# 0xPolygonZero/proof-protocol-decoder

Hardware: AMD Instinct MI355X
Metric: txn-proofs/sec (whole node), 256-txn synthetic block (higher is better)
Workload: dtype u64 (Goldilocks field)

## Files before the change

### include/bpg.h

```cpp
#ifndef BPG_H
#define BPG_H
#include <stddef.h>
#include <stdint.h>

#ifdef __cplusplus
extern "C" {
#endif

typedef enum {
  BP_OK = 0,
  BP_ERR_ABORTED = -1,
  BP_ERR_INVALID_INPUT = -2,
  BP_ERR_RANGE = -3,
  BP_ERR_DEVICE = -4,
  BP_ERR_VERIFY = -5,
  BP_ERR_UNSUPPORTED = -6
} bp_status;

const char* bp_last_error(void);
const char* bp_version(void);
int bp_device_count(void);
int bp_use_blocking_sync(int device);
int bp_host_wait_mode(int device);

// ... 127 lines not shown
typedef struct bp_plonk_layout {
  uint32_t pi_len, n_paths, path_depth, path_pi0;
  uint32_t leaf_len;
} bp_plonk_layout;
int bp_plonk_constants(uint64_t seed, uint32_t log_n, const bp_plonk_layout* layout, uint64_t* d_consts_out, void* stream);
int bp_plonk_trace(const uint64_t* d_consts, uint64_t seed, const uint64_t* pi, const bp_plonk_layout* layout, const uint64_t* paths,
                   uint32_t log_n, uint64_t* d_trace_out, void* stream);

int bp_fri_fold(const uint64_t* d_values, uint32_t log_nl, uint32_t rate_bits, uint32_t arity_bits, uint64_t shift,
                const uint64_t beta[2], uint64_t* d_out, void* stream);

int bp_openings(const uint64_t* d_coeffs, uint64_t stride, uint32_t log_n, uint32_t n_cols, const uint64_t z0[2],
                const uint64_t z1[2], uint64_t* d_pw_scratch, uint64_t* d_out, void* stream);

int bp_pow_grind(const uint64_t state[12], uint32_t pos, uint32_t bits, uint64_t* nonce_out, void* stream);

typedef struct bp_stark_cfg {
  uint32_t log_n, n_cols, n_const, deg_pow, rate_bits, cap_height, num_queries, pow_bits, arity_bits,
      final_poly_bits;
} bp_stark_cfg;
int bp_stark_prove_synthetic(const bp_stark_cfg* cfg, uint64_t seed, uint64_t const_seed, int device,
                             uint8_t** out, size_t* out_len);
int bp_stark_prove_air(uint32_t air_id, const bp_stark_cfg* cfg, uint64_t seed, uint64_t const_seed, int device,
                       uint8_t** out, size_t* out_len);
int bp_stark_prove_trace(uint32_t air_id, const bp_stark_cfg* cfg, const uint64_t* d_trace, uint64_t stride,
                         const uint64_t* d_consts, const uint64_t* pub, int device, uint8_t** out, size_t* out_len);
int bp_stark_verify_air(uint32_t air_id, const bp_stark_cfg* cfg, const uint64_t* const_cap, const uint8_t* proof,
                        size_t len);
void bp_stark_public_inputs(uint64_t seed, uint64_t out[4]);
void bp_stark_public_input_list(uint64_t seed, uint64_t out[4]);
// ... 220 lines not shown
```

### proof_protocol_decoder_amd/_abi.py

```python
import ctypes as C
from ctypes import POINTER as P

vp, cp, i, sz, dbl = C.c_void_p, C.c_char_p, C.c_int, C.c_size_t, C.c_double
u8, u32, u64, i32, i64 = C.c_uint8, C.c_uint32, C.c_uint64, C.c_int32, C.c_int64
u8p, u32p, u64p, i32p, szp = P(u8), P(u32), P(u64), P(i32), P(sz)
u8pp = P(u8p)

BP_OK, BP_ERR_ABORTED, BP_ERR_INVALID_INPUT, BP_ERR_RANGE, BP_ERR_DEVICE, BP_ERR_VERIFY, BP_ERR_UNSUPPORTED = 0, -1, -2, -3, -4, -5, -6
STATUS_NAMES = {v: k for k, v in list(globals().items()) if k == "BP_OK" or k.startswith("BP_ERR_")}
BP_SET_SKIP_LINK_CHECK = 1
BP_NUM_TABLES, BP_IR_WORDS, BP_PV_WORDS = 7, 25, 13

KNOBS = ("quad_threshold", "assume_loaded", "merkle_fused", "merkle_wide", "poseidon_mx", "poseidon_mx_sets",
         "poseidon_grouped", "ntt_mx", "ntt_split", "k5_spread", "host_wait", "host_poseidon", "rec_batch",
         "witness_threads", "side_lanes")


def _u32s(*names):
    return [(n, u32) for n in names]


class AirFamily(C.Structure):
    _fields_ = _u32s("first_index", "count", "kind", "degree")

# ... 170 lines not shown
    "bp_arithmetic_div_trace": (i, [vp, u32, vp, vp]),
    "bp_arithmetic_div_layout": (i, [u32p, sz]),
    "bp_arithmetic_mod_trace": (i, [vp, u32, vp, vp]),
    "bp_arithmetic_mod_layout": (i, [u32p, sz]),
    "bp_arithmetic_shift_trace": (i, [vp, u32, vp, vp]),
    "bp_arithmetic_shift_layout": (i, [u32p, sz]),
    "bp_arithmetic_sdiv_trace": (i, [vp, u32, vp, vp]),
    "bp_arithmetic_sdiv_layout": (i, [u32p, sz]),
    "bp_arithmetic_exp_trace": (i, [vp, u32, vp, u32, vp, vp]),
    "bp_arithmetic_exp_layout": (i, [u32p, sz]),
    "bp_plonk_constants": (i, [u64, u32, P(PlonkLayout), vp, vp]),
    "bp_plonk_trace": (i, [vp, u64, u64p, P(PlonkLayout), u64p, u32, vp, vp]),
    "bp_fri_fold": (i, [vp, u32, u32, u32, u64, u64p, vp, vp]),
    "bp_openings": (i, [vp, u64, u32, u32, u64p, u64p, vp, vp, vp]),
    "bp_pow_grind": (i, [u64p, u32, u32, u64p, vp]),
    "bp_stark_prove_synthetic": (i, [_cfg, u64, u64, i] + _buf),
    "bp_stark_prove_air": (i, [u32, _cfg, u64, u64, i] + _buf),
    "bp_stark_prove_trace": (i, [u32, _cfg, vp, u64, vp, u64p, i] + _buf),
    "bp_stark_verify_air": (i, [u32, _cfg, u64p, cp, sz]),
    "bp_stark_public_inputs": (None, [u64, u64p]),
    "bp_stark_public_input_list": (None, [u64, u64p]),
    "bp_stark_verify_air_pub": (i, [u32, _cfg, u64p, u64p, cp, sz]),
    "bp_stark_prove_table_set": (i, [P(SetTable), u32, P(SetLink), u32, u32, i] + _buf),
    "bp_stark_verify_table_set": (i, [P(SetTable), u32, P(u64p), P(SetLink), u32, cp, sz]),
    "bp_check_table_set": (i, [P(SetTable), u32, P(SetLink), u32, i, P(SetReport)]),
    "bp_release_cached_memory": (None, []),
    "bp_free_buffer": (None, [u8p]),
    "bp_config_default": (None, [_conf]),
    "bp_state_build": (i, [_conf, P(vp)]),
    "bp_state_free": (None, [vp]),
# ... 54 lines not shown
```

### proof_protocol_decoder_amd/csrc/poseidon.cuh

```cuda
#pragma once
#include "gl.hpp"
#include "mx_arith.cuh"

namespace poseidon {

static __constant__ uint64_t RC[360] = {
#include "poseidon_rc.inc"
};

__device__ __forceinline__ uint64_t sbox(uint64_t x) {
  uint64_t x2 = gl::sqr(x);
  uint64_t x4 = gl::sqr(x2);
  uint64_t x3 = gl::mul(x2, x);
  return gl::mul(x3, x4);
}

template <int N>
__device__ __forceinline__ void sbox_n(uint64_t (&x)[N]) {
  uint64_t x2[N], x4[N], x3[N];
  gl::mul_n<N>(x, x, x2);
  gl::mul_n<N>(x2, x2, x4);
  gl::mul_n<N>(x2, x, x3);
  gl::mul_n<N>(x3, x4, x);
}
// ... 37 lines not shown
        L[rr] += (uint64_t)lo[(i + r) % 12] * C[i];
        H[rr] += (uint64_t)hi[(i + r) % 12] * C[i];
      }
      if (r == 0) {
        L[rr] += (uint64_t)lo[0] * 8;
        H[rr] += (uint64_t)hi[0] * 8;
      }
    }
    uint64_t out[4];
    reduce_rows<4>(L, H, out);
#pragma unroll
    for (int rr = 0; rr < 4; rr++) s[4 * g + rr] = out[rr];
  }
}

__device__ __forceinline__ void permute(uint64_t (&s)[12]) {
#pragma unroll
  for (int i = 0; i < 12; i++) s[i] = gl::add(s[i], RC[i]);
  int rnd = 0;
#pragma unroll 1
  for (int k = 0; k < 4; k++, rnd++) {
    sbox_all(s);
    mds<true>(s, RC + (rnd + 1) * 12);
  }
#pragma unroll 1
  for (int k = 0; k < 22; k++, rnd++) {
    s[0] = sbox(s[0]);
    mds<true>(s, RC + (rnd + 1) * 12);
  }
#pragma unroll 1
  for (int k = 0; k < 3; k++, rnd++) {
    sbox_all(s);
    mds<true>(s, RC + (rnd + 1) * 12);
  }
  sbox_all(s);
  mds<false>(s, nullptr);
}
// ... 93 lines not shown
```

### proof_protocol_decoder_amd/csrc/poseidon_mx.cuh

```cuda
#pragma once
#include "poseidon.cuh"
#include "poseidon_group.hpp"

namespace poseidon {
namespace mx {

using mxa::v4i;

constexpr int CIN_PER_ROUND = 4 * 24;
constexpr int CIN_WORDS = 30 * CIN_PER_ROUND;

__device__ __forceinline__ uint32_t mds_entry(uint32_t i, uint32_t k) {
  constexpr uint32_t C[12] = {17, 15, 41, 16, 2, 28, 13, 13, 39, 18, 34, 20};
  const uint32_t d = (k + 12 - i) % 12;
  uint32_t v = 0;
#pragma unroll
  for (int j = 0; j < 12; j++) v = d == (uint32_t)j ? C[j] : v;
  return v + ((i | k) == 0 ? 8u : 0u);
}

struct CinTable {
  uint32_t v[CIN_WORDS];
};
constexpr CinTable make_cin_table() {
// ... 342 lines not shown
    blo[3] = 0;
    bhi[3] = 0;
    uint64_t L[3], H[3];
#pragma unroll
    for (int g = 0; g < 3; g++) {
      const v4i A = am[g * 64];
      const v4i dl = __builtin_amdgcn_mfma_i32_16x16x64_i8(A, blo, cr[2 * g], 0, 0, 0);
      const v4i dh = __builtin_amdgcn_mfma_i32_16x16x64_i8(A, bhi, cr[2 * g + 1], 0, 0, 0);
      L[g] = planes(dl);
      H[g] = planes(dh);
    }
    reduce_rows<3>(L, H, e[m]);
  }
}

__device__ __forceinline__ void permute_grouped(uint64_t (&e)[4][3], const Ctx& c, const uint32_t* tab,
                                                const uint32_t* __restrict__ gtab) {
#pragma unroll
  for (int a = 0; a < 3; a++) {
    const uint64_t k = RC[c.kb + 4 * a];
#pragma unroll
    for (int m = 0; m < 4; m++) e[m][a] = gl::add(e[m][a], k);
  }
  int rnd = 0;
#pragma unroll 1
  for (int k = 0; k < 4; k++, rnd++) {
    sbox_full<4>(e);
    mds4_lds(e, c, rnd, tab);
  }
  grp::State s;
  grp::init_state(s);
  grp::Lanes o = grp::lanes_of(threadIdx.x & 63);
#pragma unroll 1
  for (int g = 0; g < grp::N_GROUPS; g++) grp::partial_group(s, o, e, tab, gtab, g);
  rnd = 26;
#pragma unroll 1
  for (int k = 0; k < 4; k++, rnd++) {
    sbox_full<4>(e);
    mds4_lds(e, c, rnd, tab);
  }
}

template <int NS>
__device__ __forceinline__ void permute(uint64_t (&e)[NS][3], const Ctx& c) {
#pragma unroll
  for (int a = 0; a < 3; a++) {
    const uint64_t k = RC[c.kb + 4 * a];
#pragma unroll
    for (int m = 0; m < NS; m++) e[m][a] = gl::add(e[m][a], k);
  }
  int rnd = 0;
#pragma unroll 1
  for (int k = 0; k < 4; k++, rnd++) {
    sbox_full<NS>(e);
    mds<NS>(e, c, rnd);
  }
#pragma unroll 1
  for (int k = 0; k < 22; k++, rnd++) {
    sbox_word0<NS>(e, c);
    mds<NS>(e, c, rnd);
  }
#pragma unroll 1
  for (int k = 0; k < 4; k++, rnd++) {
    sbox_full<NS>(e);
    mds<NS>(e, c, rnd);
  }
}

}
}
```

### proof_protocol_decoder_amd/csrc/prover.cpp

```cpp
#include <cstdio>
#include <cstdlib>
#include "prover.hpp"
#include "tune.hpp"
#include <algorithm>
#include <chrono>
#if defined(__x86_64__)
#include <immintrin.h>
#endif
#include <memory>
#include <mutex>
#include <unordered_map>
#include <thread>

namespace bpg {

static const uint64_t RC_HOST[360] = {
#include "poseidon_rc.inc"
};
static inline uint64_t sbox_host(uint64_t x) {
  uint64_t x2 = gl::mulc(x, x), x4 = gl::mulc(x2, x2), x3 = gl::mulc(x2, x);
  return gl::mulc(x3, x4);
}
static const uint32_t MDS_C[12] = {17, 15, 41, 16, 2, 28, 13, 13, 39, 18, 34, 20};
static inline void mds_finish_host(const uint64_t al[12], const uint64_t ah[12], uint64_t s[12]) {
// ... 67 lines not shown
      else for (int i = 0; i < 12; i++) s[i] = sbox_host(s[i]);
      mds(s);
    }
  }
}
#if defined(__x86_64__)
__attribute__((target("avx2"))) static void poseidon_host_avx2(uint64_t s[12]) { poseidon_host_body<true>(s); }
#endif
static void poseidon_host_scalar(uint64_t s[12]) { poseidon_host_body<false>(s); }
void poseidon_host(uint64_t s[12]) {
#if defined(__x86_64__)
  static const bool avx2 = __builtin_cpu_supports("avx2");
  if (avx2 && tune().host_poseidon.load(std::memory_order_relaxed) == 0) return poseidon_host_avx2(s);
#endif
  poseidon_host_scalar(s);
}
template <bool AVX2>
__attribute__((always_inline)) static inline void permutation_wires_body(uint64_t (&s)[12], uint64_t* w) {
  namespace pk = air::plonk;
  for (int rnd = 0; rnd < 30; rnd++) {
    for (int i = 0; i < 12; i++) s[i] = gl::addc(s[i], RC_HOST[rnd * 12 + i]);
    const bool full = rnd < 4 || rnd >= 26;
    if (rnd >= 1 && rnd <= 3) std::memcpy(w + pk::H_FULL1 + 12 * (rnd - 1), s, sizeof(s));
    else if (rnd >= 4 && rnd <= 25) w[pk::H_PART + rnd - 4] = s[0];
    else if (rnd >= 26) std::memcpy(w + pk::H_FULL2 + 12 * (rnd - 26), s, sizeof(s));
    if (full) for (int i = 0; i < 12; i++) s[i] = sbox_host(s[i]);
    else s[0] = sbox_host(s[0]);
#if defined(__x86_64__)
    if (AVX2) mds_host_avx2(s);
    else
// ... 763 lines not shown
        if (k < L.final_len) {
          P[b][L.final_poly + 2 * k] = c0;
          P[b][L.final_poly + 2 * k + 1] = c1;
        } else if (c0 || c1) {
          return fail(BP_ERR_INVALID_INPUT, "FRI final polynomial has a non-zero tail: the witness violates the AIR");
        }
      }
      ch[b].observe(P[b] + L.final_poly, 2 * (size_t)L.final_len);
    }
  }
  if (w.aborted()) return fail(BP_ERR_ABORTED, "aborted before proof of work");

  {
    PowArgs pa[MAX_LOCKSTEP] = {};
    for (uint32_t b = 0; b < B; b++) {
      ch[b].pow_state(pa[b].state, &pa[b].pos);
      pa[b].bits = cfg.pow_bits;
    }
    unsigned long long res[MAX_LOCKSTEP];
    for (uint32_t b = 0; b < B; b++) res[b] = 0;
    if (cfg.pow_bits) {
      const uint32_t batch0 = (uint32_t)std::min<uint64_t>(1u << 20, std::max<uint64_t>(1u << 12, (uint64_t)1 << (cfg.pow_bits ? cfg.pow_bits - 1 : 0)));
      uint32_t batch = batch0, n_batches = 0;
      BPG_HIP(hipMemsetAsync(w.d_pow_result, 0xFF, 8 * MAX_LOCKSTEP, st));
      for (uint64_t base = 0;;) {
        for (int k = 0; k < 4; k++) {
          if (++n_batches > 8) batch = std::min<uint32_t>(1u << 20, batch * 2);
          for (uint32_t b = 0; b < B; b++) pa[b].base = base;
          TRY(launch_pow(pa, B, batch, w.d_pow_result, st));
          base += batch;
        }
        BPG_HIP(hipMemcpyAsync(w.pinned, w.d_pow_result, 8 * B, hipMemcpyDeviceToHost, st));
        TRY(w.wait());
        bool all = true;
        for (uint32_t b = 0; b < B; b++) {
          res[b] = reinterpret_cast<const unsigned long long*>(w.pinned)[b];
          all = all && res[b] != ~0ULL;
        }
        if (all) break;
        if (w.aborted()) return fail(BP_ERR_ABORTED, "aborted during proof of work");
        if (base > ((uint64_t)1 << 44)) return fail(BP_ERR_DEVICE, "proof of work search exhausted");
      }
    }
    for (uint32_t b = 0; b < B; b++) {
      const uint64_t nonce = res[b];
      P[b][L.pow] = nonce;
// ... 52 lines not shown
```

### proof_protocol_decoder_amd/csrc/prover.hpp

```cpp
#pragma once
#include <atomic>
#include <cstdint>
#include <cstring>
#include <random>
#include <vector>
#include "common.hpp"
#include "gl.hpp"
#include "stark_kernels.hpp"
#include "arg_ring.hpp"
#include "air_program.hpp"

namespace bpg {

void poseidon_host(uint64_t s[12]);
void hash_no_pad_host(const uint64_t* in, size_t len, uint64_t out[4]);
void poseidon_hash_rows(const uint64_t* in, size_t n, std::vector<uint64_t>* rows, uint64_t digest[4]);
void poseidon_merkle_rows(const uint64_t leaf[4], uint64_t index, const uint64_t* siblings, uint32_t depth, uint64_t* rows,
                          uint64_t root[4]);

class Challenger {
 public:
  Challenger() { std::memset(this, 0, sizeof(*this)); }
  void observe(uint64_t e) {
    n_out_ = 0;
// ... 20 lines not shown
    for (unsigned i = 0; i < n_in_; i++) st[i] = in_[i];
    *pos = n_in_;
  }

 private:
  void duplex() {
    for (unsigned i = 0; i < n_in_; i++) state_[i] = in_[i];
    n_in_ = 0;
    poseidon_host(state_);
    std::memcpy(out_, state_, 8 * sizeof(uint64_t));
    n_out_ = 8;
  }
  uint64_t state_[12], in_[8], out_[8];
  unsigned n_in_, n_out_;
};

struct FreshChallenges {
  std::mt19937_64 g{((uint64_t)std::random_device{}() << 32) ^ std::random_device{}()};
  uint64_t operator()() {
    uint64_t a;
    do a = g() % gl::P; while (a < 2);
    return a;
  }
};

struct StarkCfg {
  uint32_t log_n, n_cols, n_const, deg_pow, rate_bits, cap_height, num_queries, pow_bits, arity_bits,
      final_poly_bits;
  uint32_t air_id = air::SYNTHETIC;
};
// ... 104 lines not shown
```

### proof_protocol_decoder_amd/csrc/stark_api.cpp

```cpp
#include <algorithm>
#include <cstdlib>
#include <cstring>
#include <vector>
#include "caller_table.hpp"

using namespace bpg;

namespace {
constexpr uint32_t LONE_PI_LEN = 4;
void lone_public_input_list(uint64_t seed, uint64_t out[LONE_PI_LEN]) {
  for (uint64_t j = 0; j < LONE_PI_LEN; j++) {
    uint64_t z = (seed ^ ((0x50 + j) << 32)) + 0x9E3779B97F4A7C15ULL;
    z = (z ^ (z >> 30)) * 0xBF58476D1CE4E5B9ULL;
    z = (z ^ (z >> 27)) * 0x94D049BB133111EBULL;
    out[j] = gl::canon(z ^ (z >> 31));
  }
}
int prove_lone(Worker& w, const CallerTable& t, uint8_t** out, size_t* out_len) {
  Challenger ch;
  Committed consts, trace;
  const uint64_t* d_values = nullptr;
  int rc = commit_caller_table(w, ch, t, &consts, &trace, &d_values);
  if (rc) return rc;
  Ctl ctl;
// ... 393 lines not shown
  FriLayerArgs fa{};
  if ((rc = fri_layer_args(log_nl, rate_bits, arity_bits, shift, &fa))) return rc;
  fa.values = d_values; fa.out = d_out; fa.digests = nullptr;
  fa.beta = gl::Ext{beta[0], beta[1]};
  return launch_fri_fold(fa, as_stream(stream));
}
BPG_ABI_CATCH("bp_fri_fold")

int bp_pow_grind(const uint64_t state[12], uint32_t pos, uint32_t bits, uint64_t* nonce_out, void* stream) try {
  if (!state || !nonce_out) return fail(BP_ERR_INVALID_INPUT, "bp_pow_grind: null argument");
  if (pos >= 8 || bits == 0 || bits > 40) return fail(BP_ERR_INVALID_INPUT, "bp_pow_grind: pos must be a rate word, bits in 1..40");
  hipStream_t st = as_stream(stream);
  DeviceBuf res_buf;
  BPG_HIP(hipMalloc(&res_buf.p, 8));
  unsigned long long* d_res = res_buf.as<unsigned long long>();
  PowArgs pa{};
  for (int i = 0; i < 12; i++) pa.state[i] = state[i];
  pa.pos = pos; pa.bits = bits;
  int rc = BP_OK;
  unsigned long long res = ~0ULL;
  if (hipMemsetAsync(d_res, 0xFF, 8, st) != hipSuccess) rc = fail(BP_ERR_DEVICE, "hipMemsetAsync failed");
  uint32_t batch = (uint32_t)std::min<uint64_t>(1u << 20, std::max<uint64_t>(1u << 12, (uint64_t)2 << bits));
  for (uint64_t base = 0; rc == BP_OK; base += batch, batch = std::min<uint32_t>(1u << 20, batch * 2)) {
    pa.base = base;
    if ((rc = launch_pow(pa, batch, d_res, st))) break;
    if (hipMemcpyAsync(&res, d_res, 8, hipMemcpyDeviceToHost, st) != hipSuccess || hipStreamSynchronize(st) != hipSuccess) {
      rc = fail(BP_ERR_DEVICE, "bp_pow_grind: copy back failed");
      break;
    }
    if (res != ~0ULL) break;
    if (base > ((uint64_t)1 << 44)) rc = fail(BP_ERR_DEVICE, "proof of work search exhausted");
  }
  if (rc == BP_OK) *nonce_out = res;
  return rc;
}
BPG_ABI_CATCH("bp_pow_grind")

int bp_openings(const uint64_t* d_coeffs, uint64_t stride, uint32_t log_n, uint32_t n_cols, const uint64_t z0[2],
                const uint64_t z1[2], uint64_t* d_pw_scratch, uint64_t* d_out, void* stream) try {
  if (!n_cols) return BP_OK;
  if (!d_coeffs || !z0 || !d_pw_scratch || !d_out) return fail(BP_ERR_INVALID_INPUT, "bp_openings: null argument");
  if (log_n > 30 || stride < ((uint64_t)1 << log_n)) return fail(BP_ERR_INVALID_INPUT, "bp_openings: bad shape");
  const uint64_t* zz[2] = {z0, z1 ? z1 : z0};
  for (int k = 0; k < 2; k++)
    if (zz[k][0] >= gl::P || zz[k][1] >= gl::P) return fail(BP_ERR_INVALID_INPUT, "bp_openings: non-canonical point");
  hipStream_t st = as_stream(stream);
  const uint32_t n_points = z1 ? 2 : 1;
  int rc = launch_power_vectors(d_pw_scratch, log_n, gl::Ext{z0[0], z0[1]}, gl::Ext{zz[1][0], zz[1][1]}, n_points, st);
  if (rc) return rc;
  return launch_openings(d_coeffs, stride, log_n, n_cols, d_pw_scratch, n_points, d_out, st);
}
// ... 4 lines not shown
```

### proof_protocol_decoder_amd/csrc/stark_kernels.hip

```cpp
#include "common.hpp"
#include "gl.hpp"
#include "poseidon.cuh"
#include "poseidon_mx.cuh"
#include "stark_kernels.hpp"
#include "arg_ring.hpp"
#include "quotient_dev.cuh"
#include "air_program.hpp"

namespace {

using gl::Ext;
using namespace bpg::k5;

__device__ __forceinline__ uint64_t splitmix64(uint64_t x) {
  uint64_t z = x + 0x9E3779B97F4A7C15ULL;
  z = (z ^ (z >> 30)) * 0xBF58476D1CE4E5B9ULL;
  z = (z ^ (z >> 27)) * 0x94D049BB133111EBULL;
  return z ^ (z >> 31);
}
__device__ __forceinline__ uint64_t rnd(uint64_t seed, uint64_t col, uint64_t row) {
  return gl::canon(splitmix64(seed ^ (col << 32) ^ row));
}
__device__ __forceinline__ uint64_t pow_e(uint64_t t, uint32_t e) {
  return e == 3 ? gl::mulc(gl::mulc(t, t), t) : t;
// ... 1137 lines not shown
      }
    }
  }
  const Ext bx = gl::scale(a.beta, x_inv);
  Ext acc = gl::ext(0);
#pragma unroll
  for (int i = 15; i >= 0; i--) {
    const int slot = ((i & 1) << 3) | ((i & 2) << 1) | ((i & 4) >> 1) | ((i & 8) >> 3);
    acc = gl::add(gl::mul(acc, bx), Ext{c0[slot], c1[slot]});
  }
  acc = gl::scale(acc, a.arity_inv);
  a.out[2 * id] = acc.c0;
  a.out[2 * id + 1] = acc.c1;
}

__global__ void __launch_bounds__(256) pow_grind_kernel(bpg::ArgPtr<bpg::PowArgs> args, unsigned long long* result) {
  BPG_ARG_BATCH(bpg::PowArgs, args);
  const bpg::PowArgs& a = batch[blockIdx.z];
  result += blockIdx.z;
  if (__hip_atomic_load(result, __ATOMIC_RELAXED, __HIP_MEMORY_SCOPE_AGENT) < a.base + blockIdx.x * (uint64_t)blockDim.x) return;
  const uint64_t cand = a.base + blockIdx.x * (uint64_t)blockDim.x + threadIdx.x;
  uint64_t s[12];
#pragma unroll
  for (int k = 0; k < 12; k++) s[k] = a.state[k];
  s[a.pos] = cand;
  poseidon::permute(s);
  if ((gl::canon(s[7]) >> (64 - a.bits)) == 0) atomicMin(result, (unsigned long long)cand);
}
template <bool GR>
__global__ void __launch_bounds__(256) __attribute__((amdgpu_waves_per_eu(3)))
pow_grind_mx_kernel(bpg::ArgPtr<bpg::PowArgs> args, unsigned long long* result, const uint32_t* __restrict__ gtab) {
  BPG_ARG_BATCH(bpg::PowArgs, args);
  const bpg::PowArgs& a = batch[blockIdx.z];
  result += blockIdx.z;
  __shared__ uint32_t beaten;
  if (threadIdx.x == 0)
    beaten = __hip_atomic_load(result, __ATOMIC_RELAXED, __HIP_MEMORY_SCOPE_AGENT) < a.base + (uint64_t)blockIdx.x * 256;
  __syncthreads();
  if (beaten) return;
  __shared__ __attribute__((aligned(16))) uint32_t cin[GR ? poseidon::mx::CIN_GROUPED_WORDS : poseidon::mx::CIN_WORDS];
  __shared__ __attribute__((aligned(16))) uint32_t gt[GR ? poseidon::mx::grp::TABLE_WORDS : 4];
  if constexpr (GR) {
    poseidon::mx::build_cin_grouped(cin);
    poseidon::mx::grp::load_tables(gt, gtab);
  } else {
    poseidon::mx::build_cin(cin);
  }
  __syncthreads();
  const poseidon::mx::Ctx c = poseidon::mx::make_ctx(cin);
  const uint64_t cand0 = a.base + ((uint64_t)blockIdx.x * 4 + (threadIdx.x >> 6)) * 64 + (threadIdx.x & 15);
  uint64_t e[4][3];
#pragma unroll
  for (int s = 0; s < 3; s++) {
    uint64_t w = a.state[4 * s];
#pragma unroll
    for (int q = 1; q < 4; q++) w = c.kb == (uint32_t)q ? a.state[4 * s + q] : w;
    const bool mine = c.kb + 4 * s == a.pos;
#pragma unroll
    for (int m = 0; m < 4; m++) e[m][s] = mine ? cand0 + 16 * m : w;
  }
  if constexpr (GR) poseidon::mx::permute_grouped(e, c, gt, gtab);
  else poseidon::mx::permute<4>(e, c);
  if (c.kb == 3) {
#pragma unroll
    for (int m = 0; m < 4; m++)
      if ((gl::canon(e[m][1]) >> (64 - a.bits)) == 0) atomicMin(result, (unsigned long long)(cand0 + 16 * m));
  }
}

__global__ void __launch_bounds__(256) query_initial_kernel(bpg::ArgPtr<bpg::QueryArgs> args) {
  if (gridDim.x * gridDim.y * gridDim.z <= 64) __builtin_amdgcn_s_setprio(3);
  const bpg::QueryArgs& a = *(const bpg::QueryArgs*)args;
  const uint32_t b = blockIdx.x / a.n_queries, q = blockIdx.x % a.n_queries, o = blockIdx.y;
  const uint64_t x = a.x_index[blockIdx.x];
  const bpg::QueryOracle& orc = a.proof[b].oracle[o];
  const uint32_t log_rows = a.log_n + a.rate_bits;
  const uint32_t i = gl::bitrev((uint32_t)x, log_rows);
  const uint64_t pos = ((uint64_t)(i & ((1u << a.rate_bits) - 1)) << a.log_n) + (i >> a.rate_bits);
  uint64_t* out = a.proof[b].out;
  if (o == 0 && threadIdx.x == 0) out[(uint64_t)q * a.query_words] = x;
  uint64_t* w = out + (uint64_t)q * a.query_words + orc.out_offset;
// ... 359 lines not shown
    else fri_layer_leaf_mx_kernel<1><<<dim3(ceil_div(n, 64), 1, batch), 256, 0, st>>>(ab);
  } else if (n * batch < quad_threshold()) fri_layer_leaf_quad_kernel<<<dim3(ceil_div(n * 4, 256), 1, batch), 256, 0, st>>>(ab);
  else fri_layer_leaf_kernel<<<dim3(ceil_div(n, 256), 1, batch), 256, 0, st>>>(ab);
  BPG_LAUNCH_CHECK();
  return BP_OK;
}
int launch_fri_fold(const FriLayerArgs* a, uint32_t batch, hipStream_t st) {
  if (int rc = check_batch(batch)) return rc;
  uint64_t n = (uint64_t)1 << (a[0].log_nl - a[0].arity_bits + a[0].rate_bits);
  BPG_ARG_BLOCKS(ab, a, batch, st);
  KernelTimer kt(PROF_FRI_FOLD, st, 16.0 * (double)n * ((1 << a[0].arity_bits) + 1) * batch, true);
  BPG_LAUNCH_TIMED(kt, fri_fold_kernel, dim3(ceil_div(n, 256), 1, batch), 256, 0, st, ab);
  BPG_LAUNCH_CHECK();
  return BP_OK;
}
int launch_pow(const PowArgs* a, uint32_t batch, uint32_t n_candidates, unsigned long long* d_result, hipStream_t st) {
  if (int rc = check_batch(batch)) return rc;
  BPG_ARG_BLOCKS(ab, a, batch, st);
  const dim3 grid(n_candidates / 256, 1, batch);
  if (poseidon_mx()) {
    const uint32_t* gtab = group_tables();
    if (gtab) pow_grind_mx_kernel<true><<<grid, 256, 0, st>>>(ab, d_result, gtab);
    else pow_grind_mx_kernel<false><<<grid, 256, 0, st>>>(ab, d_result, nullptr);
  } else
    pow_grind_kernel<<<grid, 256, 0, st>>>(ab, d_result);
  BPG_LAUNCH_CHECK();
  return BP_OK;
}
int launch_query_initial(const QueryArgs& a, uint32_t batch, uint32_t n_oracles, hipStream_t st) {
  if (int rc = check_batch(batch)) return rc;
  if (!a.n_queries || a.n_queries * batch > MAX_BATCH_QUERIES) return fail(BP_ERR_INVALID_INPUT, "query launch: %u x %u indices, at most %u", a.n_queries, batch, MAX_BATCH_QUERIES);
  dim3 grid(a.n_queries * batch, n_oracles);
  const QueryArgs* ab = nullptr;
  if (int rc = arg_put(st, &a, 1, &ab)) return rc;
  query_initial_kernel<<<grid, 256, 0, st>>>(arg_ptr(ab));
  BPG_LAUNCH_CHECK();
  return BP_OK;
}
int launch_query_layers(const QueryLayerArgs& a, uint32_t batch, uint32_t n_layers, hipStream_t st) {
  if (!n_layers) return BP_OK;
// ... 13 lines not shown
```

### proof_protocol_decoder_amd/csrc/stark_kernels.hpp

```cpp
#pragma once
#include <hip/hip_runtime.h>
#include <cstdint>
#include "air.hpp"
#include "gl.hpp"

namespace bpg {

struct Ctl {
  uint64_t v[4];
  uint64_t pub[4] = {0, 0, 0, 0};
};

constexpr uint32_t MAX_BATCH = 8;
constexpr uint32_t MAX_LOCKSTEP = 24;
int arg_ring_put(hipStream_t st, const void* blocks, size_t bytes, const void** dev);
template <class A>
using ArgPtr = const __attribute__((address_space(4))) A*;
template <class A>
inline ArgPtr<A> arg_ptr(const A* dev) { return (ArgPtr<A>)dev; }
#define BPG_ARG_BATCH(T, args) const T* __restrict__ batch = (const T*)(args)
template <class A>
inline int arg_put(hipStream_t st, const A* a, uint32_t n, const A** dev) {
  const void* d = nullptr;
  const int rc = arg_ring_put(st, a, sizeof(A) * n, &d);
// ... 78 lines not shown
  uint64_t g_t[16];
  gl::Ext y[3], z[3], alpha_shift[3];
};
struct FriLayerArgs {
  const uint64_t* values;
  uint64_t* out;
  uint64_t* digests;
  const uint64_t* tw_nl_inv;
  uint32_t log_nl, rate_bits, arity_bits;
  uint64_t g_t_inv[16];
  uint64_t wa_inv_pow[16];
  uint64_t arity_inv;
  gl::Ext beta;
};
struct PowArgs {
  uint64_t state[12];
  uint64_t base;
  uint32_t pos, bits;
};
struct QueryOracle {
  const uint64_t *lde, *digests;
  uint64_t stride;
  uint32_t n_cols, out_offset;
};
constexpr uint32_t MAX_BATCH_QUERIES = 672;
struct QueryProof {
  uint64_t* out;
  QueryOracle oracle[4];
  uint64_t* first_leaf = nullptr;
};
struct QueryArgs {
  uint64_t x_index[MAX_BATCH_QUERIES];
  uint64_t query_words;
  uint32_t log_n, rate_bits, cap_height, n_queries;
// ... 58 lines not shown
                                hipStream_t st, gl::Ext z2 = gl::Ext{1, 0}) {
  const PowerVecArgs a{d_out, {z0, z1, z2}};
  return launch_power_vectors(&a, 1, log_n, n_points, st);
}
int launch_alpha_pows(const AlphaPowArgs* a, uint32_t batch, uint32_t count, hipStream_t st);
int launch_openings(const uint64_t* d_coeffs, uint64_t stride, uint32_t log_n, uint32_t n_cols,
                    const uint64_t* d_pw, uint32_t n_points, uint64_t* d_out, hipStream_t st);
int launch_openings_multi(const OpenMulti* m, uint32_t batch, hipStream_t st);
int launch_combine_partial_multi(const CombineMulti* m, uint32_t batch, uint32_t total_chunks, hipStream_t st);
int launch_combine_all(const CombineMulti* m, uint32_t batch, uint64_t* const* d_g, hipStream_t st);
int launch_combine_reduce(const CombineReduceArgs* a, uint32_t batch, uint32_t n_chunks, uint32_t log_n, hipStream_t st);
int launch_fri_init(const FriInitArgs* a, uint32_t batch, hipStream_t st);
int launch_fri_layer_leaves(const FriLayerArgs* a, uint32_t batch, hipStream_t st);
int launch_fri_fold(const FriLayerArgs* a, uint32_t batch, hipStream_t st);
inline int launch_fri_fold(const FriLayerArgs& a, hipStream_t st) { return launch_fri_fold(&a, 1, st); }
int launch_pow(const PowArgs* a, uint32_t batch, uint32_t n_candidates, unsigned long long* d_result, hipStream_t st);
inline int launch_pow(const PowArgs& a, uint32_t n_candidates, unsigned long long* d_result, hipStream_t st) {
  return launch_pow(&a, 1, n_candidates, d_result, st);
}
int launch_query_initial(const QueryArgs& a, uint32_t batch, uint32_t n_oracles, hipStream_t st);
int launch_query_layers(const QueryLayerArgs& a, uint32_t batch, uint32_t n_layers, hipStream_t st);

int init_ntt_kernels();
int get_table(int kind, uint32_t log_n, uint32_t rate_bits, const uint64_t** out);
int intt_nat2br(const uint64_t* in, uint64_t in_stride, uint64_t* out, uint64_t out_stride, uint32_t log_n,
                uint32_t n_cols, bool inverse, hipStream_t st);
int ntt_br2nat(const uint64_t* in, uint64_t in_stride, uint64_t* out, uint64_t out_stride, uint64_t coset_stride,
               uint32_t log_n, uint32_t n_cols, uint32_t n_cosets, const uint64_t* scale, bool inverse,
               hipStream_t st);
const uint32_t* group_tables();
int merkle_upper_levels(uint64_t* d_digests, uint32_t log_leaves, uint32_t cap_height, hipStream_t st,
                        uint64_t* mirror, bool* mirrored, uint32_t batch = 1, uint64_t dig_bstride = 0);
int merkle_commit_cols(const uint64_t* d_lde, uint64_t lde_stride, uint32_t n_cols, uint32_t log_n, uint32_t rate_bits,
// ... 5 lines not shown
```

### proof_protocol_decoder_amd/ops.py

```python
import contextlib
import ctypes as C

import numpy as np
import torch

from ._lib import KNOBS, StarkCfg, call_for_buffer, check, lib, own

NTT_FWD_BR2NAT, NTT_INV_NAT2BR, NTT_FWD_NAT, NTT_INV_NAT = 0, 1, 2, 3


def _stream():
    return torch.cuda.current_stream().cuda_stream


_tuned_active = False


@contextlib.contextmanager
def tuned(**knobs):
    global _tuned_active
    if _tuned_active:
        raise RuntimeError("ops.tuned() inside ops.tuned(): name all the knobs in one call")
    unknown = sorted(set(knobs) - set(KNOBS))
    if unknown:
# ... 310 lines not shown
    _require_cuda(coeffs)
    n_cols, n = coeffs.shape
    pw = torch.empty(4 * n, dtype=torch.int64, device=coeffs.device)
    out = torch.zeros((n_cols, 4), dtype=torch.int64, device=coeffs.device)
    a0 = (C.c_uint64 * 2)(int(z0[0]), int(z0[1]))
    a1 = (C.c_uint64 * 2)(int(z1[0]), int(z1[1])) if z1 is not None else None
    check(own().bp_openings(coeffs.data_ptr(), n, n.bit_length() - 1, n_cols, a0, a1, pw.data_ptr(), out.data_ptr(),
                            _stream()))
    return out


def pow_grind(state, pos, bits):
    nonce = C.c_uint64()
    check(own().bp_pow_grind((C.c_uint64 * 12)(*[int(x) for x in state]), pos, bits, C.byref(nonce), _stream()))
    return nonce.value


def merkle_commit(lde, log_n, rate_bits, cap_height):
    _require_cuda(lde)
    n_cols, rows = lde.shape
    assert rows == 1 << (log_n + rate_bits)
    words = own().bp_merkle_digest_words(log_n + rate_bits, cap_height)
    dig = torch.empty((words // 4, 4), dtype=torch.int64, device=lde.device)
    check(own().bp_merkle_commit(lde.data_ptr(), rows, n_cols, log_n, rate_bits, cap_height, dig.data_ptr(),
                                 _stream()))
    return dig


def stark_cfg(log_n, n_cols, n_const=0, deg_pow=1, rate_bits=1, cap_height=4, num_queries=84, pow_bits=16,
              arity_bits=4, final_poly_bits=5):
# ... 193 lines not shown
```

Before: 39.01.

## Precompute PoW round-0 sbox on host and restructure grind launch windows

The host now precomputes the first round-constant add and S-box for the eleven fixed state words, so the grind kernels only compute the S-box for the nonce word and skip round 0's full S-box. The PoW search loop now issues one larger launch per host round trip instead of four smaller ones. It also replaces the 3D grid with a 1D grid whose workgroups interleave proofs in slices, so lockstep proofs advance together. Debug entry points for searching and dumping word 7 are added, and a null-check on word7 now sits in the hot path.

```diff
diff --git a/include/bpg.h b/include/bpg.h
--- a/include/bpg.h
+++ b/include/bpg.h
@@ -165,6 +165,9 @@
                 const uint64_t z1[2], uint64_t* d_pw_scratch, uint64_t* d_out, void* stream);
 
 int bp_pow_grind(const uint64_t state[12], uint32_t pos, uint32_t bits, uint64_t* nonce_out, void* stream);
+int bp_debug_pow_search(const uint64_t* states, const uint32_t* pos, uint32_t batch, uint32_t bits, uint64_t base,
+                        uint32_t log_window, uint32_t log_slice, uint64_t* result, uint32_t* round_trips, void* stream);
+int bp_debug_pow_word7(const uint64_t state[12], uint32_t pos, uint64_t base, uint32_t window, uint64_t* d_out, void* stream);
 
 typedef struct bp_stark_cfg {
   uint32_t log_n, n_cols, n_const, deg_pow, rate_bits, cap_height, num_queries, pow_bits, arity_bits,
diff --git a/proof_protocol_decoder_amd/_abi.py b/proof_protocol_decoder_amd/_abi.py
--- a/proof_protocol_decoder_amd/_abi.py
+++ b/proof_protocol_decoder_amd/_abi.py
@@ -208,6 +208,8 @@
     "bp_fri_fold": (i, [vp, u32, u32, u32, u64, u64p, vp, vp]),
     "bp_openings": (i, [vp, u64, u32, u32, u64p, u64p, vp, vp, vp]),
     "bp_pow_grind": (i, [u64p, u32, u32, u64p, vp]),
+    "bp_debug_pow_search": (i, [u64p, u32p, u32, u32, u64, u32, u32, u64p, u32p, vp]),
+    "bp_debug_pow_word7": (i, [u64p, u32, u64, u32, vp, vp]),
     "bp_stark_prove_synthetic": (i, [_cfg, u64, u64, i] + _buf),
     "bp_stark_prove_air": (i, [u32, _cfg, u64, u64, i] + _buf),
     "bp_stark_prove_trace": (i, [u32, _cfg, vp, u64, vp, u64p, i] + _buf),
diff --git a/proof_protocol_decoder_amd/csrc/poseidon.cuh b/proof_protocol_decoder_amd/csrc/poseidon.cuh
--- a/proof_protocol_decoder_amd/csrc/poseidon.cuh
+++ b/proof_protocol_decoder_amd/csrc/poseidon.cuh
@@ -75,13 +75,16 @@
   }
 }
 
+template <bool SBOX0_DONE = false>
 __device__ __forceinline__ void permute(uint64_t (&s)[12]) {
+  if constexpr (!SBOX0_DONE) {
 #pragma unroll
-  for (int i = 0; i < 12; i++) s[i] = gl::add(s[i], RC[i]);
+    for (int i = 0; i < 12; i++) s[i] = gl::add(s[i], RC[i]);
+  }
   int rnd = 0;
 #pragma unroll 1
   for (int k = 0; k < 4; k++, rnd++) {
-    sbox_all(s);
+    if (!SBOX0_DONE || k) sbox_all(s);
     mds<true>(s, RC + (rnd + 1) * 12);
   }
 #pragma unroll 1
diff --git a/proof_protocol_decoder_amd/csrc/poseidon_mx.cuh b/proof_protocol_decoder_amd/csrc/poseidon_mx.cuh
--- a/proof_protocol_decoder_amd/csrc/poseidon_mx.cuh
+++ b/proof_protocol_decoder_amd/csrc/poseidon_mx.cuh
@@ -380,58 +380,63 @@
   }
 }
 
+template <bool SBOX0_DONE = false>
 __device__ __forceinline__ void permute_grouped(uint64_t (&e)[4][3], const Ctx& c, const uint32_t* tab,
                                                 const uint32_t* __restrict__ gtab) {
-#pragma unroll
-  for (int a = 0; a < 3; a++) {
-    const uint64_t k = RC[c.kb + 4 * a];
-#pragma unroll
-    for (int m = 0; m < 4; m++) e[m][a] = gl::add(e[m][a], k);
+  if constexpr (!SBOX0_DONE) {
+#pragma unroll
+    for (int a = 0; a < 3; a++) {
+      const uint64_t k = RC[c.kb + 4 * a];
+#pragma unroll
+      for (int m = 0; m < 4; m++) e[m][a] = gl::add(e[m][a], k);
+    }
   }
   int rnd = 0;
+#pragma unroll 1
+  for (int k = 0; k < 4; k++, rnd++) {
+    if (!SBOX0_DONE || k) sbox_full<4>(e);
+    mds4_lds(e, c, rnd, tab);
+  }
+  grp::State s;
+  grp::init_state(s);
+  grp::Lanes o = grp::lanes_of(threadIdx.x & 63);
+#pragma unroll 1
+  for (int g = 0; g < grp::N_GROUPS; g++) grp::partial_group(s, o, e, tab, gtab, g);
+  rnd = 26;
 #pragma unroll 1
   for (int k = 0; k < 4; k++, rnd++) {
     sbox_full<4>(e);
     mds4_lds(e, c, rnd, tab);
   }
-  grp::State s;
-  grp::init_state(s);
-  grp::Lanes o = grp::lanes_of(threadIdx.x & 63);
-#pragma unroll 1
-  for (int g = 0; g < grp::N_GROUPS; g++) grp::partial_group(s, o, e, tab, gtab, g);
-  rnd = 26;
+}
+
+template <int NS, bool SBOX0_DONE = false>
+__device__ __forceinline__ void permute(uint64_t (&e)[NS][3], const Ctx& c) {
+  if constexpr (!SBOX0_DONE) {
+#pragma unroll
+    for (int a = 0; a < 3; a++) {
+      const uint64_t k = RC[c.kb + 4 * a];
+#pragma unroll
+      for (int m = 0; m < NS; m++) e[m][a] = gl::add(e[m][a], k);
+    }
+  }
+  int rnd = 0;
 #pragma unroll 1
   for (int k = 0; k < 4; k++, rnd++) {
-    sbox_full<4>(e);
-    mds4_lds(e, c, rnd, tab);
-  }
-}
-
-template <int NS>
-__device__ __forceinline__ void permute(uint64_t (&e)[NS][3], const Ctx& c) {
-#pragma unroll
-  for (int a = 0; a < 3; a++) {
-    const uint64_t k = RC[c.kb + 4 * a];
-#pragma unroll
-    for (int m = 0; m < NS; m++) e[m][a] = gl::add(e[m][a], k);
-  }
-  int rnd = 0;
+    if (!SBOX0_DONE || k) sbox_full<NS>(e);
+    mds<NS>(e, c, rnd);
+  }
+#pragma unroll 1
+  for (int k = 0; k < 22; k++, rnd++) {
+    sbox_word0<NS>(e, c);
+    mds<NS>(e, c, rnd);
+  }
 #pragma unroll 1
   for (int k = 0; k < 4; k++, rnd++) {
     sbox_full<NS>(e);
     mds<NS>(e, c, rnd);
   }
-#pragma unroll 1
-  for (int k = 0; k < 22; k++, rnd++) {
-    sbox_word0<NS>(e, c);
-    mds<NS>(e, c, rnd);
-  }
-#pragma unroll 1
-  for (int k = 0; k < 4; k++, rnd++) {
-    sbox_full<NS>(e);
-    mds<NS>(e, c, rnd);
-  }
-}
-
-}
-}
+}
+
+}
+}
diff --git a/proof_protocol_decoder_amd/csrc/prover.cpp b/proof_protocol_decoder_amd/csrc/prover.cpp
--- a/proof_protocol_decoder_amd/csrc/prover.cpp
+++ b/proof_protocol_decoder_amd/csrc/prover.cpp
@@ -105,6 +105,13 @@
   if (avx2 && tune().host_poseidon.load(std::memory_order_relaxed) == 0) return poseidon_host_avx2(s);
 #endif
   poseidon_host_scalar(s);
+}
+void pow_args(const uint64_t state[12], uint32_t pos, uint32_t bits, PowArgs* a) {
+  *a = PowArgs{};
+  for (uint32_t k = 0; k < 12; k++)
+    if (k != pos) a->round0[k] = sbox_host(gl::addc(gl::canon(state[k]), RC_HOST[k]));
+  a->pos = pos;
+  a->bits = bits;
 }
 template <bool AVX2>
 __attribute__((always_inline)) static inline void permutation_wires_body(uint64_t (&s)[12], uint64_t* w) {
@@ -898,22 +905,21 @@
   {
     PowArgs pa[MAX_LOCKSTEP] = {};
     for (uint32_t b = 0; b < B; b++) {
-      ch[b].pow_state(pa[b].state, &pa[b].pos);
-      pa[b].bits = cfg.pow_bits;
+      uint64_t state[12];
+      uint32_t pos;
+      ch[b].pow_state(state, &pos);
+      pow_args(state, pos, cfg.pow_bits, &pa[b]);
     }
     unsigned long long res[MAX_LOCKSTEP];
     for (uint32_t b = 0; b < B; b++) res[b] = 0;
     if (cfg.pow_bits) {
-      const uint32_t batch0 = (uint32_t)std::min<uint64_t>(1u << 20, std::max<uint64_t>(1u << 12, (uint64_t)1 << (cfg.pow_bits ? cfg.pow_bits - 1 : 0)));
-      uint32_t batch = batch0, n_batches = 0;
       BPG_HIP(hipMemsetAsync(w.d_pow_result, 0xFF, 8 * MAX_LOCKSTEP, st));
-      for (uint64_t base = 0;;) {
-        for (int k = 0; k < 4; k++) {
-          if (++n_batches > 8) batch = std::min<uint32_t>(1u << 20, batch * 2);
-          for (uint32_t b = 0; b < B; b++) pa[b].base = base;
-          TRY(launch_pow(pa, B, batch, w.d_pow_result, st));
-          base += batch;
-        }
+      uint64_t base = 0;
+      for (uint32_t trip = 0;; trip++) {
+        const uint32_t window = pow_window(cfg.pow_bits, trip);
+        for (uint32_t b = 0; b < B; b++) pa[b].base = base;
+        TRY(launch_pow(pa, B, window, w.d_pow_result, st));
+        base += window;
         BPG_HIP(hipMemcpyAsync(w.pinned, w.d_pow_result, 8 * B, hipMemcpyDeviceToHost, st));
         TRY(w.wait());
         bool all = true;
diff --git a/proof_protocol_decoder_amd/csrc/prover.hpp b/proof_protocol_decoder_amd/csrc/prover.hpp
--- a/proof_protocol_decoder_amd/csrc/prover.hpp
+++ b/proof_protocol_decoder_amd/csrc/prover.hpp
@@ -58,6 +58,8 @@
   uint64_t state_[12], in_[8], out_[8];
   unsigned n_in_, n_out_;
 };
+
+void pow_args(const uint64_t state[12], uint32_t pos, uint32_t bits, PowArgs* a);
 
 struct FreshChallenges {
   std::mt19937_64 g{((uint64_t)std::random_device{}() << 32) ^ std::random_device{}()};
diff --git a/proof_protocol_decoder_amd/csrc/stark_api.cpp b/proof_protocol_decoder_amd/csrc/stark_api.cpp
--- a/proof_protocol_decoder_amd/csrc/stark_api.cpp
+++ b/proof_protocol_decoder_amd/csrc/stark_api.cpp
@@ -431,9 +431,8 @@
   DeviceBuf res_buf;
   BPG_HIP(hipMalloc(&res_buf.p, 8));
   unsigned long long* d_res = res_buf.as<unsigned long long>();
-  PowArgs pa{};
-  for (int i = 0; i < 12; i++) pa.state[i] = state[i];
-  pa.pos = pos; pa.bits = bits;
+  PowArgs pa;
+  pow_args(state, pos, bits, &pa);
   int rc = BP_OK;
   unsigned long long res = ~0ULL;
   if (hipMemsetAsync(d_res, 0xFF, 8, st) != hipSuccess) rc = fail(BP_ERR_DEVICE, "hipMemsetAsync failed");
@@ -452,6 +451,59 @@
   return rc;
 }
 BPG_ABI_CATCH("bp_pow_grind")
+
+int bp_debug_pow_search(const uint64_t* states, const uint32_t* pos, uint32_t batch, uint32_t bits, uint64_t base,
+                        uint32_t log_window, uint32_t log_slice, uint64_t* result, uint32_t* round_trips, void* stream) try {
+  if (!states || !pos || !result) return fail(BP_ERR_INVALID_INPUT, "bp_debug_pow_search: null argument");
+  if (batch < 1 || batch > MAX_LOCKSTEP) return fail(BP_ERR_INVALID_INPUT, "bp_debug_pow_search: 1..%u proofs", MAX_LOCKSTEP);
+  if (bits == 0 || bits > 40) return fail(BP_ERR_INVALID_INPUT, "bp_debug_pow_search: bits in 1..40");
+  if (log_window && (log_window < 8 || log_window > 22)) return fail(BP_ERR_INVALID_INPUT, "bp_debug_pow_search: log_window 0 or 8..22");
+  PowArgs pa[MAX_LOCKSTEP];
+  for (uint32_t b = 0; b < batch; b++) {
+    if (pos[b] >= 12) return fail(BP_ERR_INVALID_INPUT, "bp_debug_pow_search: pos is a state word, 0..11");
+    pow_args(states + 12 * b, pos[b], bits, &pa[b]);
+  }
+  hipStream_t st = as_stream(stream);
+  DeviceBuf res_buf;
+  BPG_HIP(hipMalloc(&res_buf.p, 8 * batch));
+  unsigned long long* d_res = res_buf.as<unsigned long long>();
+  BPG_HIP(hipMemcpyAsync(d_res, result, 8 * batch, hipMemcpyHostToDevice, st));
+  uint32_t trips = 0;
+  for (;; trips++) {
+    bool all = true;
+    if (trips) {
+      BPG_HIP(hipMemcpyAsync(result, d_res, 8 * batch, hipMemcpyDeviceToHost, st));
+      BPG_HIP(hipStreamSynchronize(st));
+    }
+    for (uint32_t b = 0; b < batch; b++) all = all && result[b] != ~0ULL;
+    if (all) break;
+    if (base > ((uint64_t)1 << 44)) return fail(BP_ERR_DEVICE, "proof of work search exhausted");
+    const uint32_t window = log_window ? 1u << log_window : pow_window(bits, trips);
+    for (uint32_t b = 0; b < batch; b++) pa[b].base = base;
+    if (int rc = launch_pow(pa, batch, window, d_res, st, log_slice)) return rc;
+    base += window;
+  }
+  if (round_trips) *round_trips = trips;
+  return BP_OK;
+}
+BPG_ABI_CATCH("bp_debug_pow_search")
+
+int bp_debug_pow_word7(const uint64_t state[12], uint32_t pos, uint64_t base, uint32_t window, uint64_t* d_out, void* stream) try {
+  if (!state || !d_out) return fail(BP_ERR_INVALID_INPUT, "bp_debug_pow_word7: null argument");
+  if (pos >= 12) return fail(BP_ERR_INVALID_INPUT, "bp_debug_pow_word7: pos is a state word, 0..11");
+  hipStream_t st = as_stream(stream);
+  DeviceBuf res_buf;
+  BPG_HIP(hipMalloc(&res_buf.p, 8));
+  BPG_HIP(hipMemsetAsync(res_buf.p, 0xFF, 8, st));
+  PowArgs pa;
+  pow_args(state, pos, 1, &pa);
+  pa.base = base;
+  pa.word7 = d_out;
+  if (int rc = launch_pow(pa, window, res_buf.as<unsigned long long>(), st)) return rc;
+  BPG_HIP(hipStreamSynchronize(st));
+  return BP_OK;
+}
+BPG_ABI_CATCH("bp_debug_pow_word7")
 
 int bp_openings(const uint64_t* d_coeffs, uint64_t stride, uint32_t log_n, uint32_t n_cols, const uint64_t z0[2],
                 const uint64_t z1[2], uint64_t* d_pw_scratch, uint64_t* d_out, void* stream) try {
diff --git a/proof_protocol_decoder_amd/csrc/stark_kernels.hip b/proof_protocol_decoder_amd/csrc/stark_kernels.hip
--- a/proof_protocol_decoder_amd/csrc/stark_kernels.hip
+++ b/proof_protocol_decoder_amd/csrc/stark_kernels.hip
@@ -1175,28 +1175,42 @@
   a.out[2 * id + 1] = acc.c1;
 }
 
-__global__ void __launch_bounds__(256) pow_grind_kernel(bpg::ArgPtr<bpg::PowArgs> args, unsigned long long* result) {
+struct PowWorkgroup {
+  uint32_t proof;
+  uint64_t offset;
+};
+__device__ __forceinline__ PowWorkgroup pow_workgroup(uint32_t n_proofs, uint32_t log_wps) {
+  const uint32_t j = blockIdx.x & ((1u << log_wps) - 1), t = blockIdx.x >> log_wps, slice = t / n_proofs;
+  return PowWorkgroup{t - slice * n_proofs, (((uint64_t)slice << log_wps) + j) * 256};
+}
+__global__ void __launch_bounds__(256)
+pow_grind_kernel(bpg::ArgPtr<bpg::PowArgs> args, unsigned long long* result, uint32_t n_proofs, uint32_t log_wps) {
   BPG_ARG_BATCH(bpg::PowArgs, args);
-  const bpg::PowArgs& a = batch[blockIdx.z];
-  result += blockIdx.z;
-  if (__hip_atomic_load(result, __ATOMIC_RELAXED, __HIP_MEMORY_SCOPE_AGENT) < a.base + blockIdx.x * (uint64_t)blockDim.x) return;
-  const uint64_t cand = a.base + blockIdx.x * (uint64_t)blockDim.x + threadIdx.x;
+  const PowWorkgroup wg = pow_workgroup(n_proofs, log_wps);
+  const bpg::PowArgs& a = batch[wg.proof];
+  result += wg.proof;
+  if (!a.word7 && __hip_atomic_load(result, __ATOMIC_RELAXED, __HIP_MEMORY_SCOPE_AGENT) < a.base + wg.offset) return;
+  const uint64_t cand = a.base + wg.offset + threadIdx.x;
+  const uint64_t x = poseidon::sbox(gl::add(cand, poseidon::RC[a.pos]));
   uint64_t s[12];
 #pragma unroll
-  for (int k = 0; k < 12; k++) s[k] = a.state[k];
-  s[a.pos] = cand;
-  poseidon::permute(s);
-  if ((gl::canon(s[7]) >> (64 - a.bits)) == 0) atomicMin(result, (unsigned long long)cand);
+  for (int k = 0; k < 12; k++) s[k] = a.pos == (uint32_t)k ? x : a.round0[k];
+  poseidon::permute<true>(s);
+  const uint64_t w7 = gl::canon(s[7]);
+  if (a.word7) a.word7[wg.offset + threadIdx.x] = w7;
+  if ((w7 >> (64 - a.bits)) == 0) atomicMin(result, (unsigned long long)cand);
 }
 template <bool GR>
 __global__ void __launch_bounds__(256) __attribute__((amdgpu_waves_per_eu(3)))
-pow_grind_mx_kernel(bpg::ArgPtr<bpg::PowArgs> args, unsigned long long* result, const uint32_t* __restrict__ gtab) {
+pow_grind_mx_kernel(bpg::ArgPtr<bpg::PowArgs> args, unsigned long long* result, const uint32_t* __restrict__ gtab,
+                    uint32_t n_proofs, uint32_t log_wps) {
   BPG_ARG_BATCH(bpg::PowArgs, args);
-  const bpg::PowArgs& a = batch[blockIdx.z];
-  result += blockIdx.z;
+  const PowWorkgroup wg = pow_workgroup(n_proofs, log_wps);
+  const bpg::PowArgs& a = batch[wg.proof];
+  result += wg.proof;
   __shared__ uint32_t beaten;
   if (threadIdx.x == 0)
-    beaten = __hip_atomic_load(result, __ATOMIC_RELAXED, __HIP_MEMORY_SCOPE_AGENT) < a.base + (uint64_t)blockIdx.x * 256;
+    beaten = !a.word7 && __hip_atomic_load(result, __ATOMIC_RELAXED, __HIP_MEMORY_SCOPE_AGENT) < a.base + wg.offset;
   __syncthreads();
   if (beaten) return;
   __shared__ __attribute__((aligned(16))) uint32_t cin[GR ? poseidon::mx::CIN_GROUPED_WORDS : poseidon::mx::CIN_WORDS];
@@ -1209,23 +1223,31 @@
   }
   __syncthreads();
   const poseidon::mx::Ctx c = poseidon::mx::make_ctx(cin);
-  const uint64_t cand0 = a.base + ((uint64_t)blockIdx.x * 4 + (threadIdx.x >> 6)) * 64 + (threadIdx.x & 15);
+  const uint64_t off0 = wg.offset + (threadIdx.x >> 6) * 64 + (threadIdx.x & 15), cand0 = a.base + off0;
+  uint64_t x[4];
+  const uint64_t k0 = poseidon::RC[a.pos];
+#pragma unroll
+  for (int m = 0; m < 4; m++) x[m] = gl::add(cand0 + 16 * m, k0);
+  poseidon::sbox_n<4>(x);
   uint64_t e[4][3];
 #pragma unroll
   for (int s = 0; s < 3; s++) {
-    uint64_t w = a.state[4 * s];
-#pragma unroll
-    for (int q = 1; q < 4; q++) w = c.kb == (uint32_t)q ? a.state[4 * s + q] : w;
+    uint64_t w = a.round0[4 * s];
+#pragma unroll
+    for (int q = 1; q < 4; q++) w = c.kb == (uint32_t)q ? a.round0[4 * s + q] : w;
     const bool mine = c.kb + 4 * s == a.pos;
 #pragma unroll
-    for (int m = 0; m < 4; m++) e[m][s] = mine ? cand0 + 16 * m : w;
-  }
-  if constexpr (GR) poseidon::mx::permute_grouped(e, c, gt, gtab);
-  else poseidon::mx::permute<4>(e, c);
+    for (int m = 0; m < 4; m++) e[m][s] = mine ? x[m] : w;
+  }
+  if constexpr (GR) poseidon::mx::permute_grouped<true>(e, c, gt, gtab);
+  else poseidon::mx::permute<4, true>(e, c);
   if (c.kb == 3) {
 #pragma unroll
-    for (int m = 0; m < 4; m++)
-      if ((gl::canon(e[m][1]) >> (64 - a.bits)) == 0) atomicMin(result, (unsigned long long)(cand0 + 16 * m));
+    for (int m = 0; m < 4; m++) {
+      const uint64_t w7 = gl::canon(e[m][1]);
+      if (a.word7) a.word7[off0 + 16 * m] = w7;
+      if ((w7 >> (64 - a.bits)) == 0) atomicMin(result, (unsigned long long)(cand0 + 16 * m));
+    }
   }
 }
 
@@ -1615,16 +1637,23 @@
   BPG_LAUNCH_CHECK();
   return BP_OK;
 }
-int launch_pow(const PowArgs* a, uint32_t batch, uint32_t n_candidates, unsigned long long* d_result, hipStream_t st) {
-  if (int rc = check_batch(batch)) return rc;
+constexpr uint32_t POW_SLICE_LOG = 12;
+int launch_pow(const PowArgs* a, uint32_t batch, uint32_t window, unsigned long long* d_result, hipStream_t st, uint32_t log_slice) {
+  if (int rc = check_batch(batch)) return rc;
+  if (window < 256 || window > POW_WINDOW_MAX || (window & (window - 1)))
+    return fail(BP_ERR_INVALID_INPUT, "launch_pow: a window of %u candidates (a power of two, 256 .. %u)", window, POW_WINDOW_MAX);
+  if (!log_slice) log_slice = POW_SLICE_LOG;
+  if (log_slice < 8 || log_slice > 22) return fail(BP_ERR_INVALID_INPUT, "launch_pow: slices of 2^%u candidates", log_slice);
   BPG_ARG_BLOCKS(ab, a, batch, st);
-  const dim3 grid(n_candidates / 256, 1, batch);
+  uint32_t log_wps = 0;
+  while (log_wps < log_slice - 8 && (512u << log_wps) <= window) log_wps++;
+  const dim3 grid(batch * (window / 256));
   if (poseidon_mx()) {
     const uint32_t* gtab = group_tables();
-    if (gtab) pow_grind_mx_kernel<true><<<grid, 256, 0, st>>>(ab, d_result, gtab);
-    else pow_grind_mx_kernel<false><<<grid, 256, 0, st>>>(ab, d_result, nullptr);
+    if (gtab) pow_grind_mx_kernel<true><<<grid, 256, 0, st>>>(ab, d_result, gtab, batch, log_wps);
+    else pow_grind_mx_kernel<false><<<grid, 256, 0, st>>>(ab, d_result, nullptr, batch, log_wps);
   } else
-    pow_grind_kernel<<<grid, 256, 0, st>>>(ab, d_result);
+    pow_grind_kernel<<<grid, 256, 0, st>>>(ab, d_result, batch, log_wps);
   BPG_LAUNCH_CHECK();
   return BP_OK;
 }
diff --git a/proof_protocol_decoder_amd/csrc/stark_kernels.hpp b/proof_protocol_decoder_amd/csrc/stark_kernels.hpp
--- a/proof_protocol_decoder_amd/csrc/stark_kernels.hpp
+++ b/proof_protocol_decoder_amd/csrc/stark_kernels.hpp
@@ -1,5 +1,6 @@
 #pragma once
 #include <hip/hip_runtime.h>
+#include <algorithm>
 #include <cstdint>
 #include "air.hpp"
 #include "gl.hpp"
@@ -116,10 +117,16 @@
   gl::Ext beta;
 };
 struct PowArgs {
-  uint64_t state[12];
+  uint64_t round0[12];
   uint64_t base;
   uint32_t pos, bits;
-};
+  uint64_t* word7 = nullptr;
+};
+constexpr uint32_t POW_WINDOW_MAX = 1u << 22;
+inline uint32_t pow_window(uint32_t bits, uint32_t round_trip) {
+  const uint64_t w0 = 4 * std::min<uint64_t>(1u << 20, std::max<uint64_t>(1u << 12, (uint64_t)1 << (bits ? bits - 1 : 0)));
+  return (uint32_t)std::min<uint64_t>(POW_WINDOW_MAX, w0 << (round_trip < 2 ? 0 : std::min(round_trip - 1, 10u)));
+}
 struct QueryOracle {
   const uint64_t *lde, *digests;
   uint64_t stride;
@@ -208,9 +215,9 @@
 int launch_fri_layer_leaves(const FriLayerArgs* a, uint32_t batch, hipStream_t st);
 int launch_fri_fold(const FriLayerArgs* a, uint32_t batch, hipStream_t st);
 inline int launch_fri_fold(const FriLayerArgs& a, hipStream_t st) { return launch_fri_fold(&a, 1, st); }
-int launch_pow(const PowArgs* a, uint32_t batch, uint32_t n_candidates, unsigned long long* d_result, hipStream_t st);
-inline int launch_pow(const PowArgs& a, uint32_t n_candidates, unsigned long long* d_result, hipStream_t st) {
-  return launch_pow(&a, 1, n_candidates, d_result, st);
+int launch_pow(const PowArgs* a, uint32_t batch, uint32_t window, unsigned long long* d_result, hipStream_t st, uint32_t log_slice = 0);
+inline int launch_pow(const PowArgs& a, uint32_t window, unsigned long long* d_result, hipStream_t st) {
+  return launch_pow(&a, 1, window, d_result, st);
 }
 int launch_query_initial(const QueryArgs& a, uint32_t batch, uint32_t n_oracles, hipStream_t st);
 int launch_query_layers(const QueryLayerArgs& a, uint32_t batch, uint32_t n_layers, hipStream_t st);
diff --git a/proof_protocol_decoder_amd/ops.py b/proof_protocol_decoder_amd/ops.py
--- a/proof_protocol_decoder_amd/ops.py
+++ b/proof_protocol_decoder_amd/ops.py
@@ -348,6 +348,22 @@
     nonce = C.c_uint64()
     check(own().bp_pow_grind((C.c_uint64 * 12)(*[int(x) for x in state]), pos, bits, C.byref(nonce), _stream()))
     return nonce.value
+
+
+def pow_search(states, pos, bits, base=0, result=None, log_window=0, log_slice=0):
+    n = len(states)
+    words = (C.c_uint64 * n)(*([2 ** 64 - 1] * n if result is None else [int(x) for x in result]))
+    trips = C.c_uint32()
+    check(own().bp_debug_pow_search((C.c_uint64 * (12 * n))(*[int(x) for s in states for x in s]),
+                                    (C.c_uint32 * n)(*[int(p) for p in pos]), n, bits, base, log_window, log_slice, words,
+                                    C.byref(trips), _stream()))
+    return list(words), trips.value
+
+
+def pow_word7(state, pos, base, window):
+    out = torch.empty(window, dtype=torch.int64, device="cuda")
+    check(own().bp_debug_pow_word7((C.c_uint64 * 12)(*[int(x) for x in state]), pos, base, window, out.data_ptr(), _stream()))
+    return out
 
 
 def merkle_commit(lde, log_n, rate_bits, cap_height):
```

Result: no change. 39.15, median of 6 (+0.4%).
